# airl-iisc/MRFP

Measured on AMD Instinct MI355X. Metric: train images/sec, higher is better.
Workload: dtype bf16; 1 GPU; resnet-101 DeepLabV3+ + MRFP+ (HRFP+NP+ on, HRFP re-drawn every step), 768x768, 16 images/GPU, fwd+bwd+SGD, synthetic 19-class, random-init weights; global_batch=16, parallelism=dp1

## Files before the change

### include/mrfp_hip.h

```cpp
#ifndef MRFP_HIP_H
#define MRFP_HIP_H

#include <stdint.h>

#ifdef __cplusplus
extern "C" {
#endif

typedef enum { MRFP_F32 = 0, MRFP_BF16 = 1, MRFP_F16 = 2 } mrfp_dtype;

int mrfp_version(void);
const char* mrfp_last_error(void);

int64_t mrfp_stats_nslab(int64_t B, int64_t Ho);

int mrfp_stats_fwd(const void* x, int dtype, int64_t B, int64_t Ho, int64_t Wo, int64_t C,
                   int64_t Hs, int64_t Ws, const int32_t* tabH, const int32_t* tabW,
                   float* ws, void* stream);

int mrfp_stats_bwd(const void* dy, const void* x, const void* y, const float* mean,
                   const float* fA, const float* fS, int per_image, int dtype, int64_t B, int64_t Ho, int64_t Wo, int64_t C,
                   int64_t Hs, int64_t Ws, const int32_t* tabH, const int32_t* tabW,
                   float* ws, void* stream);
int mrfp_stats_bwd_mask(const void* dy, const void* x, const void* mask, const float* mean, int per_image, int dtype, int64_t B,
// ... 117 lines not shown
                  int64_t sstride, const void* addend, float* colstats, void* stream);
int mrfp_conv_fwd_act(const void* x, const void* wpack, const float* bias, void* y, int dtype,
                      int64_t B, int64_t H, int64_t W, int64_t C, int64_t N, int64_t ldy, int64_t R, int64_t S,
                      int64_t Ho, int64_t Wo, int64_t stride, int64_t pad_h, int64_t pad_w, int64_t dil,
                      int64_t sstride, const void* addend, int act, void* stream);
int mrfp_pack_weight_folded(const float* w, void* wf, const float* conv_bias, const float* bn_weight, const float* bn_bias,
                            const float* running_mean, const float* running_var, float eps, float* bias_out, int dtype,
                            int64_t N, int64_t C, int64_t R, int64_t S, int64_t Npad, int64_t Cpad, void* stream);
int mrfp_pack_weights_folded_batched(const void* jobs, const int64_t* prefix, int64_t njobs, int64_t total, int dtype, void* stream);
int mrfp_conv_stats_layout(int dtype, int64_t B, int64_t H, int64_t W, int64_t C, int64_t N, int64_t ldy, int64_t R, int64_t S,
                           int64_t Ho, int64_t Wo, int64_t stride, int64_t pad_h, int64_t pad_w, int64_t dil, int64_t sstride, int wstats,
                           int64_t* out);
int64_t mrfp_conv_stats_block_rows(int dtype, int64_t B, int64_t H, int64_t W, int64_t C, int64_t N, int64_t R, int64_t S, int64_t Ho,
                                   int64_t Wo, int64_t stride, int64_t pad_h, int64_t pad_w, int64_t dil, int64_t sstride);
int mrfp_conv_single_launch(int64_t B, int64_t image_bytes);
int mrfp_conv_fwd_wstats(const void* x, const void* wpack, const float* bias, void* y, int dtype,
                         int64_t B, int64_t H, int64_t W, int64_t C, int64_t N, int64_t ldy, int64_t R, int64_t S,
                         int64_t Ho, int64_t Wo, int64_t stride, int64_t pad_h, int64_t pad_w, int64_t dil,
                         const uint8_t* rowweight, float* colstats, void* stream);
int mrfp_conv_fwd_gated(const void* x, const void* wpack, const float* bias, void* y, int dtype,
                        int64_t B, int64_t H, int64_t W, int64_t C, int64_t N, int64_t ldy, int64_t R, int64_t S,
                        int64_t Ho, int64_t Wo, int64_t stride, int64_t pad_h, int64_t pad_w, int64_t dil,
                        int64_t sstride, const void* addend, const void* addend_mask, void* stream);
int mrfp_debug_clock_stamps(int family, uint64_t* out, int64_t n);
int64_t mrfp_conv_wgrad_ws_bytes(int64_t M, int64_t N, int64_t Q);
int mrfp_conv_wgrad(const void* x, const void* dy, float* dw, void* ws, int dtype,
                    int64_t B, int64_t H, int64_t W, int64_t C, int64_t Ctrue, int64_t N, int64_t ldn,
                    int64_t R, int64_t S, int64_t Ho, int64_t Wo, int64_t stride, int64_t pad_h, int64_t pad_w,
                    int64_t dil, void* stream);
int64_t mrfp_conv_wgrad_group_max(void);
int64_t mrfp_conv_wgrad_grouped_ws_bytes(int64_t M, int64_t N, int64_t Q, int64_t count);
int mrfp_conv_wgrad_plan(int dtype, int64_t B, int64_t H, int64_t W, int64_t C, int64_t N, int64_t ldn, int64_t R, int64_t S, int64_t Ho,
                         int64_t Wo, int64_t stride, int64_t pad_h, int64_t pad_w, int64_t dil, int64_t count, int64_t* out);
int mrfp_conv_wgrad_grouped(const void* const* xs, const void* const* dys, float* const* dws, int64_t count, void* ws, int dtype,
                            int64_t B, int64_t H, int64_t W, int64_t C, int64_t Ctrue, int64_t N, int64_t ldn,
                            int64_t R, int64_t S, int64_t Ho, int64_t Wo, int64_t stride, int64_t pad_h, int64_t pad_w,
                            int64_t dil, void* stream);
int mrfp_nchw_to_nhwc_pad(const float* x, void* y, int dtype, int64_t B, int64_t C, int64_t H, int64_t W,
                          int64_t Cpad, void* stream);

int mrfp_sgd_step(float* p, const float* g, float* m, int64_t n, float lr, float momentum,
                  float weight_decay, float gscale, int first, void* stream);

int64_t mrfp_grad_check_nblocks(int64_t n);
int mrfp_grad_check(const float* g, int64_t n, float gscale, void* ws, void* state, int dynamic, float growth,
                    float backoff, int growth_interval, float max_norm, void* stream);
// ... 70 lines not shown
```

### mrfp_amd/conv.py

```python
from __future__ import annotations

import collections
import ctypes
import os as _os
import warnings
import weakref
from typing import Any, NamedTuple, Optional

import torch

from . import _lib
from ._lib import call, dt, ptr, stream
from .ops import CL, GRAD_DEFERRED, _chk, channel_sums, empty_cl, grad_sink, notify_grad, wgrad_workspace, zeros_cl
from .ops import _inside_autograd_engine as _in_backward

_PACKS = {}
FUSE_STATS = [_os.environ.get("MRFP_FUSE_STATS", "1") != "0"]


class ConvStats(NamedTuple):
    final: torch.Tensor
    final_count: int
    elements: int
    rows: torch.Tensor
    row_blocks: int
    block_rows: int
    resize_plan: Any
    version: int


WSTATS = [_os.environ.get("MRFP_WSTATS", "1") != "0"]
WSTATS_HITS = [0]
_EPOCH = [0]


def invalidate_packs():
    _EPOCH[0] += 1
# ... 546 lines not shown
        else:
            call("mrfp_conv_fwd", ptr(x), ptr(pk.wf), ptr(pk.bias), ptr(y), dt(x), B, H, W, Cphys, Nphys, Nphys, R, S,
                 Ho, Wo, stride, pad_h, pad_w, dil, 1, None, ptr(stats), stream())
        ctx.save_for_backward(x, weight, bias)
        ctx.cfg = (stride, pad_h, pad_w, dil, Nphys, Ho, Wo)
        ctx.set_materialize_grads(False)
        if want_skip:
            return y, x.view_as(x)
        return y

    @staticmethod
    def backward(ctx, dy, dskip=None):
        x, weight, bias = ctx.saved_tensors
        cell = getattr(ctx, "_mrfp_cell", None)
        if cell is not None and cell[1]:
            g = getattr(dskip, "_mrfp_gate", None) if dskip is not None else None
            if g is None or g[1] != dskip._version:
                raise _lib.MrfpHipError("a gated skip gradient reached its convolution without its gate: the skip alias was "
                                        "also consumed by an operator outside mrfp_amd.ops (set MRFP_GATED_SKIP=0)")
            cell[1] = False
        if dy is None:
            return (ungate(dskip),) + (None,) * 10
        stride, pad_h, pad_w, dil, Nphys, Ho, Wo = ctx.cfg
        dy = _chk(dy, "dy")
        B, Cphys, H, W = x.shape
        N, C, R, S = weight.shape
        dx = dw = db = None
        if ctx.needs_input_grad[0]:
            pk = get_pack(weight, bias, x.dtype, Cphys, Nphys)
            dx = empty_cl(B, Cphys, H, W, x.dtype, x.device)
            gate = None
            if dskip is not None:
                g = getattr(dskip, "_mrfp_gate", None)
                if g is not None:
                    if (g[1] == dskip._version and dskip.dtype == x.dtype and x.element_size() == 2
                            and Cphys % 8 == 0 and dskip.shape == dx.shape and dskip.is_contiguous(memory_format=CL)):
                        gate = g[0]
                    else:
                        dskip = ungate(dskip)
                dskip = _chk(dskip, "dskip")
                if dskip.dtype != x.dtype:
                    dskip = dskip.to(x.dtype)
            _lib.NOTE[0] = (N, C)
            if gate is not None:
                call("mrfp_conv_fwd_gated", ptr(dy), ptr(pk.wd), None, ptr(dx), dt(dy), B, Ho, Wo, Nphys, Cphys, Cphys, R, S, H, W,
                     1, dil * (R - 1) - pad_h, dil * (S - 1) - pad_w, dil, stride, ptr(dskip), ptr(gate), stream())
                GATED_SKIP_HITS[0] += 1
            else:
                call("mrfp_conv_fwd", ptr(dy), ptr(pk.wd), None, ptr(dx), dt(dy), B, Ho, Wo, Nphys, Cphys, Cphys, R, S, H, W,
                     1, dil * (R - 1) - pad_h, dil * (S - 1) - pad_w, dil, stride, ptr(dskip), None, stream())
        if ctx.needs_input_grad[1]:
            sig = (x.dtype, B, H, W, Cphys, C, N, Nphys, R, S, Ho, Wo, stride, pad_h, pad_w, dil)
            sink = grad_sink(weight)
            side = _WGRADS.stream(x.device) if sink is not None else None
            if sink is not None and GROUP_WGRAD[0] and L_single(B, H, W, Cphys, Ho, Wo, Nphys, x.element_size()):
                _WGRADS.submit(sig, x, dy, sink, weight)
            elif side is not None:
                _WGRADS.ensure_callback()
                _launch_wgrads(sig, [(x, dy, sink)], side)
                notify_grad(weight)
            else:
                dw = sink if sink is not None else torch.empty((N, C, R, S), dtype=torch.float32, device=x.device)
                _launch_wgrads(sig, [(x, dy, dw)], None)
                if sink is not None:
                    notify_grad(weight)
                    dw = None
                elif dw.dtype != weight.dtype:
# ... 99 lines not shown
    R, S = weight.shape[2], weight.shape[3]
    Ho, Wo = _out_size(H, R, st, ph, dl), _out_size(W, S, st, pw, dl)
    L = _lib.lib()
    single = bool(L.mrfp_conv_single_launch(B, H * W * Cphys * x.element_size()))
    plan, wtab, stats = stat_resize, None, None
    if plan is not None and WSTATS[0] and FUSE_STATS[0] and single and (plan.Hs, plan.Ws) == (Ho, Wo) and R * S > 1:
        wtab = plan.multiplicity(B)
    if wtab is not None or (bias is None and FUSE_STATS[0] and single):
        lay = (ctypes.c_int64 * 5)()
        rc = L.mrfp_conv_stats_layout(dt(x), B, H, W, Cphys, Nphys, Nphys, R, S, Ho, Wo, st, ph, pw, dl, 1, int(wtab is not None), lay)
        if rc != 0:
            raise _lib.MrfpHipError("mrfp_conv_stats_layout failed (%d): %s" % (rc, L.mrfp_last_error().decode()))
        nblk, rb, rows, first, cnt = lay
        stats = torch.empty(rows * 2 * Nphys, dtype=torch.float32, device=x.device)
    if _WGRADS.callback_queued and not _in_backward():
        _WGRADS.drop_stale()
    out = _Conv2d.apply(x, weight, bias, st, ph, pw, dl, Nphys, want_skip, stats, wtab)
    y, skip = out if want_skip else (out, None)
    if skip is not None:
        skip._mrfp_skip_alias = True
        skip._mrfp_uses = [0, False]
        if y.grad_fn is not None:
            y.grad_fn._mrfp_cell = skip._mrfp_uses
    if stats is not None and (phys_out is not None or Nphys == N):
        final = stats[first * 2 * Nphys:(first + cnt) * 2 * Nphys]
        if wtab is not None:
            y._mrfp_colstats = ConvStats(final, cnt, B * plan.Ho * plan.Wo, stats, nblk, 0, plan, y._version)
        else:
            y._mrfp_colstats = ConvStats(final, cnt, B * Ho * Wo, stats, nblk, rb, None, y._version)
    if phys_out is None and Nphys != N:
        y = y[:, :N].contiguous(memory_format=CL)
    return (y, skip) if want_skip else y
```

### mrfp_amd/csrc/conv_pwk.hip

```cpp
#include "conv_common.hpp"

namespace mrfp {

#if MRFP_CLOCK_STAMP
__device__ unsigned long long g_phase_pwk[kStampSlots][2];
int stamps_pwk(unsigned long long* out, int n) { return hipMemcpyFromSymbol(out, HIP_SYMBOL(g_phase_pwk), (size_t)n * 16) == hipSuccess ? 0 : -1; }
struct PhaseClock {
    unsigned long long acc[8];
    unsigned long long cnt[8];
    unsigned long long last, t0, r0;
    static __device__ __forceinline__ unsigned long long now() {
        const unsigned long long t = __builtin_amdgcn_s_memtime();
        __builtin_amdgcn_s_waitcnt(0xC07F);
        return t;
    }
    __device__ __forceinline__ void start() {
#pragma unroll
        for (int k = 0; k < 8; ++k) { acc[k] = 0; cnt[k] = 0; }
        r0 = __builtin_amdgcn_s_memrealtime();
        last = t0 = now();
    }
    template <int K> __device__ __forceinline__ void lap() {
        const unsigned long long t = now();
        acc[K] += t - last;
// ... 18 lines not shown
#else
int stamps_pwk(unsigned long long*, int) { return -1; }
#define PH_START()
#define PH_LAP(k)
#define PH_FLUSH(w)
#endif


struct PkP {
    const char* x;
    const char* w;
    char* y;
    const char* addend;
    const unsigned char* addend_mask;
    float* colstats;
    int M, N, ldy;
    int tiles;
    int panels;
    int chunks;
    unsigned xbytes, wbytes, ybytes;
};

constexpr int kPkRows = 48;

template <typename T, int KQ, int NST, bool STATS, bool ADD, int ACT = 0>
__global__ __launch_bounds__(256, (KQ <= 2 ? 2 : 1)) void conv1x1_longk_kernel(PkP p) {
    constexpr int ROWB = KQ * 512;
    constexpr int STAGE = 4 * kPkRows * 128;
    constexpr int NP = 6;
    extern __shared__ __attribute__((aligned(16))) char smem[];
    const int t = threadIdx.x, lane = t & 63;
    const int wave = __builtin_amdgcn_readfirstlane(t >> 6);
    const int l15 = lane & 15, lq = lane >> 4;
    const unsigned lds0 = (unsigned)(size_t)(__attribute__((address_space(3))) char*)smem;
    const i32x4 xw = rsrc_words(p.x, p.xbytes);
    const __amdgpu_buffer_rsrc_t wr = __builtin_amdgcn_make_buffer_rsrc((void*)p.w, 0, (int)p.wbytes, 0x00020000);
    const __amdgpu_buffer_rsrc_t yr = __builtin_amdgcn_make_buffer_rsrc((void*)p.y, 0, (int)p.ybytes, 0x00020000);
    const __amdgpu_buffer_rsrc_t ar = __builtin_amdgcn_make_buffer_rsrc((void*)(p.addend ? p.addend : p.y), 0, (int)p.ybytes, 0x00020000);

    const int b = blockIdx.x, xcd = b & 7, rest = b >> 3;
    const int panel = rest % p.panels, chunk = xcd + 8 * (rest / p.panels);
    if (chunk >= p.chunks) return;
    const int per = (p.tiles + p.chunks - 1) / p.chunks;
    const int t0 = chunk * per, t1 = min(p.tiles, t0 + per);
    if (t0 >= t1) return;
    const int n0 = panel * 128 + wave * 32, nl = n0 + 8 * lq;
// ... 120 lines not shown
            u32x4 dv;
            dv.x = v.x; dv.y = v.y; dv.z = v.z; dv.w = v.w;
            __builtin_amdgcn_raw_buffer_store_b128(dv, yr, (int)(ok ? ((unsigned)m * (unsigned)p.ldy + (unsigned)nl) * 2u : kOOB), 0, 0);
        }
    }
    if constexpr (STATS) {
        float* out = p.colstats + (size_t)chunk * 2 * p.ldy;
#pragma unroll
        for (int u = 0; u < 8; ++u) {
            cs[u] = row16_sum(cs[u]);
            cq[u] = row16_sum(cq[u]);
        }
        if (l15 == 0 && nl < p.N) {
#pragma unroll
            for (int u = 0; u < 8; ++u) {
                out[nl + u] = cs[u];
                out[p.ldy + nl + u] = cq[u];
            }
        }
    }
}

constexpr int kPk2Rows = 32;

template <typename T, bool STATS, bool ADD, int ACT = 0>
__global__ __launch_bounds__(512, 2) void conv1x1_longk2_kernel(PkP p) {
    constexpr int ROWB = 2048;
    constexpr int QTR = 4 * kPk2Rows * 128;
    constexpr int PAIR = 2 * QTR;
    constexpr int NST = 4;
    constexpr int NP = 4;
    extern __shared__ __attribute__((aligned(16))) char smem[];
    char* const exch = smem + NST * PAIR;
    const int t = threadIdx.x, lane = t & 63;
    const int wave = __builtin_amdgcn_readfirstlane(t >> 6);
    const int grp = wave >> 2, wq = wave & 3;
    const int l15 = lane & 15, lq = lane >> 4;
    const unsigned lds0 = (unsigned)(size_t)(__attribute__((address_space(3))) char*)smem;
    const i32x4 xw = rsrc_words(p.x, p.xbytes);
    const __amdgpu_buffer_rsrc_t wr = __builtin_amdgcn_make_buffer_rsrc((void*)p.w, 0, (int)p.wbytes, 0x00020000);
    const __amdgpu_buffer_rsrc_t yr = __builtin_amdgcn_make_buffer_rsrc((void*)p.y, 0, (int)p.ybytes, 0x00020000);
    const __amdgpu_buffer_rsrc_t ar = __builtin_amdgcn_make_buffer_rsrc((void*)(p.addend ? p.addend : p.y), 0, (int)p.ybytes, 0x00020000);

    const int b = blockIdx.x, xcd = b & 7, rest = b >> 3;
    const int panel = rest % p.panels, chunk = xcd + 8 * (rest / p.panels);
    if (chunk >= p.chunks) return;
    const int per = (p.tiles + p.chunks - 1) / p.chunks;
    const int t0 = chunk * per, t1 = min(p.tiles, t0 + per);
    if (t0 >= t1) return;
    const int n0 = panel * 128 + wq * 32, nl = n0 + 8 * lq;
    const int total = (t1 - t0) * 2;
    PH_START();

    unsigned src[NP];
#pragma unroll
    for (int j = 0; j < NP; ++j) {
        const int pi = j * 8 + wave, qs = pi >> 4, wi = pi & 15, kb = wi >> 2, r8 = wi & 3;
        const int row = r8 * 8 + (lane >> 3);
        const int ch = (lane & 7) ^ ((row >> 1) & 7);
        src[j] = (unsigned)row * (unsigned)ROWB + (unsigned)(qs * 1024 + kb * 128 + ch * 16);
    }
    auto issue = [&](int h) {
        const int tile = t0 + (h >> 1), sst = h & 1;
        const unsigned base = (unsigned)tile * (unsigned)(kPk2Rows * ROWB) + (unsigned)(sst * 512);
        const unsigned sbase = lds0 + (unsigned)((h % NST) * PAIR);
#pragma unroll
        for (int j = 0; j < NP; ++j) {
            const int pi = j * 8 + wave, qs = pi >> 4, wi = pi & 15, kb = wi >> 2, r8 = wi & 3;
            dma16_async(xw, sbase + (unsigned)(qs * QTR + kb * (kPk2Rows * 128) + r8 * 1024), base + src[j]);
        }
    };
#pragma unroll
    for (int h = 0; h < NST - 1; ++h)
        if (h < total) issue(h);

    uint4 fw[16][2];
#pragma unroll
    for (int ks = 0; ks < 16; ++ks)
#pragma unroll
        for (int j = 0; j < 2; ++j) {
            const int n = n0 + 8 * (l15 >> 2) + 4 * j + (l15 & 3);
            fw[ks][j] = bload(wr, n < p.N ? (unsigned)n * (unsigned)ROWB + (unsigned)(grp * 1024 + ks * 64 + lq * 16) : kOOB);
        }
#pragma unroll
    for (int ks = 0; ks < 16; ++ks)
#pragma unroll
        for (int j = 0; j < 2; ++j) settle(fw[ks][j]);
    PH_LAP(0);

    float cs[8], cq[8];
#pragma unroll
    for (int u = 0; u < 8; ++u) { cs[u] = 0.f; cq[u] = 0.f; }

    int h = 0;
    for (int tile = t0; tile < t1; ++tile) {
        f32x4 acc[2][2];
        uint4 av[2];
        unsigned am[2] = {0xffu, 0xffu};
#pragma unroll
        for (int sst = 0; sst < 2; ++sst, ++h) {
            if (h + NST - 1 <= total) dma_wait<(NST - 2) * NP>();
            else dma_wait<0>();
            __builtin_amdgcn_s_barrier();
            PH_LAP(1);
            if (h + NST - 1 < total) issue(h + NST - 1);
            PH_LAP(2);
            if constexpr (ADD) {
                if (sst == 0 && grp == 0) {
#pragma unroll
                    for (int rb = 0; rb < 2; ++rb) {
                        const int m = tile * kPk2Rows + rb * 16 + l15;
                        const bool ok = m < p.M && nl < p.N;
                        av[rb] = bload(ar, ok ? ((unsigned)m * (unsigned)p.ldy + (unsigned)nl) * 2u : kOOB);
                        am[rb] = (p.addend_mask && ok) ? p.addend_mask[((size_t)m * p.ldy + nl) >> 3] : 0xffu;
                    }
                }
            }
            const char* st = smem + (h % NST) * PAIR + grp * QTR;
            uint4 fx[2][2];
            auto read_x = [&](int ks, uint4 (&f)[2]) {
                const char* ab = st + (ks >> 1) * (kPk2Rows * 128);
                const int ch = (ks & 1) * 4 + lq;
#pragma unroll
                for (int rb = 0; rb < 2; ++rb) f[rb] = *reinterpret_cast<const uint4*>(ab + lds_off(rb * 16 + l15, ch));
            };
            read_x(0, fx[0]);
#pragma unroll
            for (int ks = 0; ks < 8; ++ks) {
                if (ks + 1 < 8) read_x(ks + 1, fx[(ks + 1) & 1]);
                __builtin_amdgcn_sched_barrier(0);
#pragma unroll
                for (int rb = 0; rb < 2; ++rb)
#pragma unroll
                    for (int j = 0; j < 2; ++j) {
                        if (sst == 0 && ks == 0) {
                            const f32x4 z = {0.f, 0.f, 0.f, 0.f};
                            acc[rb][j] = z;
                        }
                        Mma16<T>::run(acc[rb][j], fw[sst * 8 + ks][j], fx[ks & 1][rb]);
                    }
                __builtin_amdgcn_sched_barrier(0);
            }
            PH_LAP(3);
        }
        f32x4* ex = reinterpret_cast<f32x4*>(exch) + (wq * 4) * 64 + lane;
        if (grp == 1) {
#pragma unroll
            for (int rb = 0; rb < 2; ++rb)
#pragma unroll
                for (int j = 0; j < 2; ++j) ex[(rb * 2 + j) * 64] = acc[rb][j];
        }
        asm volatile("s_waitcnt lgkmcnt(0)" ::: "memory");
        __builtin_amdgcn_s_barrier();
        if (grp == 0) {
#pragma unroll
            for (int rb = 0; rb < 2; ++rb) {
#pragma unroll
                for (int j = 0; j < 2; ++j) {
                    const f32x4 o = ex[(rb * 2 + j) * 64];
#pragma unroll
                    for (int e = 0; e < 4; ++e) acc[rb][j][e] += o[e];
                }
                const int m = tile * kPk2Rows + rb * 16 + l15;
                const bool ok = m < p.M && nl < p.N;
// ... 87 lines not shown

template <typename T, bool STATS, bool ADD, int ACT = 0>
static int pwk2_launch(const ConvP& c, hipStream_t st) {
    constexpr int lds = 4 * 2 * 4 * kPk2Rows * 128 + kPk2Rows * 128 * 4;
    static bool attr_set = false;
    if (!attr_set) {
        (void)hipFuncSetAttribute(reinterpret_cast<const void*>(&conv1x1_longk2_kernel<T, STATS, ADD, ACT>),
                                  hipFuncAttributeMaxDynamicSharedMemorySize, lds);
        attr_set = true;
    }
    PkP p;
    p.x = c.x; p.w = c.w; p.y = c.y; p.addend = c.addend; p.addend_mask = c.addend_mask; p.colstats = c.colstats;
    p.M = c.M; p.N = c.N; p.ldy = c.ldy;
    p.tiles = (c.M + kPk2Rows - 1) / kPk2Rows;
    p.panels = (c.N + 127) / 128;
    p.chunks = pwk_chunks(c.M, c.N, 2048);
    const int chunks = (p.chunks + 7) / 8 * 8;
    p.xbytes = c.xbytes; p.wbytes = c.wbytes; p.ybytes = (unsigned)((int64_t)c.M * c.ldy * 2);
    hipLaunchKernelGGL((conv1x1_longk2_kernel<T, STATS, ADD, ACT>), dim3((unsigned)(p.panels * chunks)), dim3(512), lds, st, p);
    MRFP_LAUNCH_CHECK();
    return 0;
}

template <typename T, int KQ, bool STATS, bool ADD, int ACT = 0>
static int pwk_launch(const ConvP& c, hipStream_t st) {
    constexpr int NST = KQ <= 2 ? 3 : 6;
    constexpr int lds = NST * 4 * kPkRows * 128;
    static bool attr_set = false;
    if (!attr_set) {
        (void)hipFuncSetAttribute(reinterpret_cast<const void*>(&conv1x1_longk_kernel<T, KQ, NST, STATS, ADD, ACT>),
                                  hipFuncAttributeMaxDynamicSharedMemorySize, lds);
        attr_set = true;
    }
    PkP p;
    p.x = c.x; p.w = c.w; p.y = c.y; p.addend = c.addend; p.addend_mask = c.addend_mask; p.colstats = c.colstats;
    p.M = c.M; p.N = c.N; p.ldy = c.ldy;
    p.tiles = (c.M + kPkRows - 1) / kPkRows;
    p.panels = (c.N + 127) / 128;
    p.chunks = pwk_chunks(c.M, c.N, c.C * 2);
    const int chunks = (p.chunks + 7) / 8 * 8;
    p.xbytes = c.xbytes; p.wbytes = c.wbytes; p.ybytes = (unsigned)((int64_t)c.M * c.ldy * 2);
    hipLaunchKernelGGL((conv1x1_longk_kernel<T, KQ, NST, STATS, ADD, ACT>), dim3((unsigned)(p.panels * chunks)), dim3(256), lds, st, p);
    MRFP_LAUNCH_CHECK();
    return 0;
}
template <typename T, int KQ>
// ... 6 lines not shown
    if (p.colstats) return pwk_launch<T, KQ, true, false>(p, st);
    if (p.addend) return pwk_launch<T, KQ, false, true>(p, st);
    return pwk_launch<T, KQ, false, false>(p, st);
}
template <typename T>
static int pwk_run_t(const ConvP& p, hipStream_t st, int act) {
    const int kq = p.C * 2 / 512;
    static const int two = env_switch("MRFP_CONV_PWK2", 1);
    if (kq == 4 && two) {
        if (act != 0) {
            if (p.colstats || p.addend_mask) return -1;
            if (act == 1) return p.addend ? pwk2_launch<T, false, true, 1>(p, st) : pwk2_launch<T, false, false, 1>(p, st);
            return p.addend ? pwk2_launch<T, false, true, 2>(p, st) : pwk2_launch<T, false, false, 2>(p, st);
        }
        if (p.colstats) return pwk2_launch<T, true, false>(p, st);
        if (p.addend) return pwk2_launch<T, false, true>(p, st);
        return pwk2_launch<T, false, false>(p, st);
    }
    return kq == 2 ? pwk_pick<T, 2>(p, st, act) : kq == 4 ? pwk_pick<T, 4>(p, st, act) : pwk_pick<T, 5>(p, st, act);
}
int pwk_run(const ConvP& p, bool is_f16, hipStream_t st, int act) { return is_f16 ? pwk_run_t<f16>(p, st, act) : pwk_run_t<bf16>(p, st, act); }

}
```

### mrfp_amd/ops.py

```python
from __future__ import annotations

import math
import os
import weakref
from functools import lru_cache
from typing import Optional, Tuple

import numpy as np
import torch

from . import _lib
from ._lib import call, dt, ptr, stream

CL = torch.channels_last

GRAD_NOTIFY = [None]
GRAD_DEFERRED = set()


def wgrad_workspace(M, N, Q, device, n=1):
    return torch.empty(int(_lib.lib().mrfp_conv_wgrad_grouped_ws_bytes(M, N, Q, n)), dtype=torch.uint8, device=device)


def grad_sink(param):
    if param is not None and getattr(param, "_mrfp_direct", False) and param.grad is not None \
            and param.grad.dtype == torch.float32 and param.grad.is_contiguous():
        return param.grad
    return None


def notify_grad(param):
    if GRAD_NOTIFY[0] is not None:
        GRAD_NOTIFY[0](param)


def to_cl(x: torch.Tensor) -> torch.Tensor:
    if x.dim() != 4:
        raise ValueError("expected a 4-D activation, got %s" % (tuple(x.shape),))
    return x.contiguous(memory_format=CL)


def empty_cl(B, C, H, W, dtype, device) -> torch.Tensor:
    return torch.empty((B, C, H, W), dtype=dtype, device=device, memory_format=CL)


def zeros_cl(B, C, H, W, dtype, device) -> torch.Tensor:
    return torch.zeros((B, H, W, C), dtype=dtype, device=device).permute(0, 3, 1, 2)


def _chk(x: torch.Tensor, name="x") -> torch.Tensor:
    if not x.is_cuda:
        raise _lib.MrfpHipError("%s must live on the GPU (got %s): the HIP path has no CPU fallback" % (name, x.device))
    uses = getattr(x, "_mrfp_uses", None)
    if uses is not None:
        uses[0] += 1
    if x.dim() != 4 or not x.is_contiguous(memory_format=CL):
        x = to_cl(x)
    return x


def _f32(t: Optional[torch.Tensor]) -> Optional[torch.Tensor]:
    if t is None:
        return None
    return t.detach().float().contiguous()


def nearest_out_size(in_size: int, scale: float) -> int:
    return int(math.floor(float(in_size) * scale))


def _nearest_table(in_size: int, out_size: int, scale: Optional[float]) -> np.ndarray:
    s = np.float32(1.0 / scale) if scale is not None else np.float32(in_size) / np.float32(out_size)
    src = np.floor(np.arange(out_size, dtype=np.float32) * s).astype(np.int64)
    return np.minimum(src, in_size - 1).astype(np.int32)


def _inverse_table(tab: np.ndarray, in_size: int) -> np.ndarray:
    lo = np.searchsorted(tab, np.arange(in_size), side="left")
# ... 206 lines not shown
    SYNC_BN_CALLS[0] += 1
    total = 0
    if count:
        key = (int(count), dist.get_world_size(group))
        total = _SYNC_BN_COUNTS.get(key)
        if total is None:
            total = _SYNC_BN_COUNTS[key] = int(round(tot[2 * C].item()))
        else:
            flag = _SYNC_BN_FLAG.get(ws.device)
            if flag is None:
                flag = _SYNC_BN_FLAG[ws.device] = torch.zeros(1, dtype=torch.int32, device=ws.device)
            flag.add_((tot[2 * C:2 * C + 1] != float(total)).to(torch.int32))
    return torch.stack([hi, lo]).contiguous(), total


ACT_NONE, ACT_RELU, ACT_RELU6 = 0, 1, 2
GATED_BN_HITS = [0]
GATED_BN = [os.environ.get("MRFP_GATED_BN", "1") != "0"]
RELU6_GATE_HITS = [0]


def _keeps_sign_mask(x, relu, res, plan):
    return bool(relu and res is not None and plan is None and SIGN_MASK[0] and x.element_size() == 2 and x.shape[1] % 8 == 0)


class _BatchNormAct(torch.autograd.Function):

    @staticmethod
    def forward(ctx, x, weight, bias, running_mean, running_var, res, training, momentum, eps, act, plan, may_sync, stats):
        relu, relu6 = act == ACT_RELU, act == ACT_RELU6
        if relu6 and (res is not None or plan is not None):
            raise _lib.MrfpHipError("BatchNorm + ReLU6 takes no residual and no resize plan")
        x = _chk(x)
        res = _chk(res, "res") if res is not None else None
        B, Ho, Wo, C, Hs, Ws, *_ = _geom(x, plan)
        dev = x.device
        w32, b32 = _f32(weight), _f32(bias)
        coef = torch.empty(4 * C, dtype=torch.float32, device=dev)
        mean, invstd, A, S = coef[0:C], coef[C:2 * C], coef[2 * C:3 * C], coef[3 * C:4 * C]
        if training:
            fused = _serving_colstats(x, C, B * Ho * Wo, plan, False)
            if fused is not None:
                ws, nb_, nslab = fused.final, 1, fused.final_count
            else:
                nslab, ws = _stats_fwd(x, plan)
                nb_ = B
            count = B * Ho * Wo
            ctx.sync = _sync_bn_group() if may_sync else None
            if ctx.sync is not None:
                ws, count = _allreduce_stats(ws, nb_ * nslab, C, count, ctx.sync)
                nb_, nslab = 1, 2
            ctx.count = count
            call("mrfp_bn_finalize", ptr(ws), nb_, nslab, count, C, ptr(w32), ptr(b32), float(eps),
                 float(momentum), ptr(running_mean), ptr(running_var), ptr(mean), ptr(invstd), ptr(A), ptr(S), stream())
        else:
            ctx.sync, ctx.count = None, B * Ho * Wo
            call("mrfp_bn_eval_coef", C, ptr(w32), ptr(b32), ptr(running_mean), ptr(running_var), float(eps),
                 ptr(A), ptr(S), stream())
            if x.requires_grad or (weight is not None and weight.requires_grad):
                mean.copy_(running_mean)
                torch.rsqrt(running_var.float() + eps, out=invstd)
        ctx.plan, ctx.act, ctx.training, ctx.has_res = plan, act, training, res is not None
        ctx.keep_y = relu and res is not None
        ctx.remask = relu and res is None
        ctx.ymask = _keeps_sign_mask(x, relu, res, plan)
        ctx.gate_skip = bool(ctx.ymask and GATED_SKIP[0] and getattr(res, "_mrfp_skip_alias", False))
        ctx.gate_ok = bool(act == ACT_NONE and res is None and plan is None and training and x.element_size() == 2 and C % 8 == 0)
        ctx.alias_uses = getattr(res, "_mrfp_uses", None)
        keep = None
        if relu6:
            y = empty_cl(B, C, Ho, Wo, x.dtype, dev)
            keep = torch.empty((B * Ho * Wo * C + 7) // 8, dtype=torch.uint8, device=dev)
            call("mrfp_affine_fwd_relu6_mask", ptr(x), ptr(y), ptr(keep), dt(x), B * Ho * Wo, C, ptr(A), ptr(S), stream())
        elif ctx.ymask:
            y = empty_cl(B, C, Ho, Wo, x.dtype, dev)
            keep = torch.empty(B * Ho * Wo * C // 8, dtype=torch.uint8, device=dev)
            call("mrfp_affine_fwd_relu_mask", ptr(x), ptr(res), ptr(y), ptr(keep), dt(x), B, Ho, Wo, C, ptr(A), ptr(S), 0, stream())
        else:
            y = _affine_fwd(x, res, A, S, False, relu, plan, stats=stats)
            if ctx.keep_y:
                keep = y
        ctx.wparam, ctx.bparam = weight, bias
        ctx.save_for_backward(x, keep, w32, mean, invstd, A, S)
        return y

    @staticmethod
    def backward(ctx, dy):
        x, keep, w32, mean, invstd, A, S = ctx.saved_tensors
        gate = None
        cell = getattr(ctx, "_mrfp_cell", None)
        g = getattr(dy, "_mrfp_gate", None)
# ... 37 lines not shown
        out = torch.empty(5 * C, dtype=torch.float32, device=dy.device)
        dw, db, P, Q, R = (out[i * C:(i + 1) * C] for i in range(5))
        dw = _grad_dest(ctx.wparam, ctx.needs_input_grad[1], dw)
        db = _grad_dest(ctx.bparam, ctx.needs_input_grad[2], db)
        call("mrfp_bn_bwd_finalize", ptr(ws), B, nslab, B * Ho * Wo, C, ptr(w32), ptr(mean), ptr(invstd),
             ptr(dw), ptr(db), ptr(P), ptr(Q), ptr(R), stream())
        if ctx.sync is not None:
            gws, _ = _allreduce_stats(ws, B * nslab, C, 0, ctx.sync)
            call("mrfp_bn_bwd_finalize", ptr(gws), 1, 2, ctx.count, C, ptr(w32), ptr(mean), ptr(invstd), None, None,
                 ptr(P), ptr(Q), ptr(R), stream())
        if not ctx.training:
            Q.zero_()
            R.zero_()
        if mask is not None:
            dx = empty_cl(B, C, Ho, Wo, dy.dtype, dy.device)
            dres = dres_out = None
            if ctx.ymask:
                if ctx.gate_skip and ctx.needs_input_grad[5] and ctx.alias_uses is not None and ctx.alias_uses[0] == 1:
                    dres = dy.view_as(dy)
                    dres._mrfp_gate = (mask, dres._version)
                    ctx.alias_uses[1] = True
                else:
                    dres = dres_out = empty_cl(B, C, Ho, Wo, dy.dtype, dy.device)
            call("mrfp_affine_bwd_mask", ptr(dy), ptr(x), ptr(mask), ptr(dx), ptr(dres_out), dt(dy), B, Ho, Wo, C, ptr(P), ptr(Q),
                 ptr(R), 0, stream())
        else:
            dx, dres = _affine_bwd(dy, x, y, P, Q, R, False, plan, ctx.has_res, x, fA, fS)
        return (dx, _grad_result(ctx.wparam, dw), _grad_result(ctx.bparam, db), None, None, dres) + (None,) * 7


RUNNING_STATS_EPOCH = [0]


def batch_norm_act(x, weight, bias, running_mean, running_var, *, training, momentum=0.1, eps=1e-5,
                   relu=False, res=None, plan=None, emit_stats=False):
    if training and running_mean is not None:
        RUNNING_STATS_EPOCH[0] += 1
    ps = _planestats_rows(x, emit_stats and plan is None and not _keeps_sign_mask(x, relu, res, plan))
    y = _BatchNormAct.apply(x, weight, bias, running_mean, running_var, res, training, momentum, eps,
                            ACT_RELU if relu else ACT_NONE, plan, True, ps[1] if ps is not None else None)
    _tag_planestats(y, ps)
    if (GATED_BN[0] and GATED_SKIP[0] and SIGN_MASK[0] and not relu and res is None and plan is None and training and y.grad_fn is not None
            and y.element_size() == 2 and y.shape[1] % 8 == 0):
        y._mrfp_skip_alias = True
        y._mrfp_uses = [0, False]
        y.grad_fn._mrfp_cell = y._mrfp_uses
    return y

# ... 1142 lines not shown
```

Measured before the change: 310.0 images/sec.

## Fuse BN-ReLU-mask backward into the following 1x1 conv's dgrad prologue

Defers the masked BN+ReLU backward elementwise pass by attaching a pending descriptor to its dx tensor. When that tensor reaches the backward of a 1x1 stride-1 K=1024 convolution, a new variant of the long-K pointwise kernel computes the BN backward on the fly while loading dy. It writes the materialized gradient once and feeds it straight into LDS for the dgrad GEMM. This removes a separate full read and write pass of the activation gradient. In exchange it adds a register-staged prologue with fewer LDS stages, use-counting and tracking machinery, and a fallback path that materializes the gradient when another op consumes it.

Result: no change. 309.9 images/sec (-0.0%).

```diff
diff --git a/include/mrfp_hip.h b/include/mrfp_hip.h
--- a/include/mrfp_hip.h
+++ b/include/mrfp_hip.h
@@ -163,6 +163,9 @@
                         int64_t B, int64_t H, int64_t W, int64_t C, int64_t N, int64_t ldy, int64_t R, int64_t S,
                         int64_t Ho, int64_t Wo, int64_t stride, int64_t pad_h, int64_t pad_w, int64_t dil,
                         int64_t sstride, const void* addend, const void* addend_mask, void* stream);
+int mrfp_conv_pw_tail_served(int dtype, int64_t B, int64_t H, int64_t W, int64_t C, int64_t N);
+int mrfp_conv_pw_tail_bwd(const void* dy, const void* x3, const void* mask, const float* P, const float* Q, const float* R, void* dx3,
+                          const void* wpack, void* y, int dtype, int64_t B, int64_t H, int64_t W, int64_t C, int64_t N, void* stream);
 int mrfp_debug_clock_stamps(int family, uint64_t* out, int64_t n);
 int64_t mrfp_conv_wgrad_ws_bytes(int64_t M, int64_t N, int64_t Q);
 int mrfp_conv_wgrad(const void* x, const void* dy, float* dw, void* ws, int dtype,
diff --git a/mrfp_amd/conv.py b/mrfp_amd/conv.py
--- a/mrfp_amd/conv.py
+++ b/mrfp_amd/conv.py
@@ -13,6 +13,7 @@
 from ._lib import call, dt, ptr, stream
 from .ops import CL, GRAD_DEFERRED, _chk, channel_sums, empty_cl, grad_sink, notify_grad, wgrad_workspace, zeros_cl
 from .ops import _inside_autograd_engine as _in_backward
+from . import ops
 
 _PACKS = {}
 FUSE_STATS = [_os.environ.get("MRFP_FUSE_STATS", "1") != "0"]
@@ -605,9 +606,18 @@
         if dy is None:
             return (ungate(dskip),) + (None,) * 10
         stride, pad_h, pad_w, dil, Nphys, Ho, Wo = ctx.cfg
-        dy = _chk(dy, "dy")
         B, Cphys, H, W = x.shape
         N, C, R, S = weight.shape
+        pend = None
+        tail = getattr(ctx, "_mrfp_tail_cell", None)
+        if tail is not None and tail[1]:
+            tail[1] = False
+            if getattr(dy, "_mrfp_pending", None) is None:
+                raise _lib.MrfpHipError("a pending tail gradient reached its convolution without its operands: the convolution's output "
+                                        "was also consumed by an operator outside mrfp_amd.ops (set MRFP_FUSE_TAIL_PW=0)")
+            if ctx.needs_input_grad[0] and dskip is None and dy.dtype == x.dtype and dy.is_contiguous(memory_format=CL):
+                pend = ops.take_pending(dy)
+        dy = _chk(dy, "dy")
         dx = dw = db = None
         if ctx.needs_input_grad[0]:
             pk = get_pack(weight, bias, x.dtype, Cphys, Nphys)
@@ -625,7 +635,11 @@
                 if dskip.dtype != x.dtype:
                     dskip = dskip.to(x.dtype)
             _lib.NOTE[0] = (N, C)
-            if gate is not None:
+            if pend is not None:
+                call("mrfp_conv_pw_tail_bwd", ptr(pend.dy), ptr(pend.x), ptr(pend.mask), ptr(pend.P), ptr(pend.Q), ptr(pend.R), ptr(dy),
+                     ptr(pk.wd), ptr(dx), dt(dy), B, Ho, Wo, Nphys, Cphys, stream())
+                ops.TAIL_PW_HITS[0] += 1
+            elif gate is not None:
                 call("mrfp_conv_fwd_gated", ptr(dy), ptr(pk.wd), None, ptr(dx), dt(dy), B, Ho, Wo, Nphys, Cphys, Cphys, R, S, H, W,
                      1, dil * (R - 1) - pad_h, dil * (S - 1) - pad_w, dil, stride, ptr(dskip), ptr(gate), stream())
                 GATED_SKIP_HITS[0] += 1
@@ -771,6 +785,10 @@
         skip._mrfp_uses = [0, False]
         if y.grad_fn is not None:
             y.grad_fn._mrfp_cell = skip._mrfp_uses
+    if (ops.FUSE_TAIL_PW[0] and not want_skip and bias is None and R == 1 and S == 1 and st == 1 and ph == 0 and pw == 0
+            and y.grad_fn is not None and x.requires_grad and L.mrfp_conv_pw_tail_served(dt(x), B, Ho, Wo, Nphys, Cphys) == 1):
+        y._mrfp_tail_cell = [0, False, weakref.ref(y)]
+        y.grad_fn._mrfp_tail_cell = y._mrfp_tail_cell
     if stats is not None and (phys_out is not None or Nphys == N):
         final = stats[first * 2 * Nphys:(first + cnt) * 2 * Nphys]
         if wtab is not None:
diff --git a/mrfp_amd/csrc/conv_pwk.hip b/mrfp_amd/csrc/conv_pwk.hip
--- a/mrfp_amd/csrc/conv_pwk.hip
+++ b/mrfp_amd/csrc/conv_pwk.hip
@@ -64,6 +64,17 @@
 };
 
 constexpr int kPkRows = 48;
+
+struct PkPre : PkP {
+    const char* a;
+    const unsigned char* mask_in;
+    char* out;
+    unsigned char* mask_out;
+    const float* c0;
+    const float* c1;
+    const float* c2;
+    unsigned mbytes;
+};
 
 template <typename T, int KQ, int NST, bool STATS, bool ADD, int ACT = 0>
 __global__ __launch_bounds__(256, (KQ <= 2 ? 2 : 1)) void conv1x1_longk_kernel(PkP p) {
@@ -230,13 +241,29 @@
 }
 
 constexpr int kPk2Rows = 32;
-
-template <typename T, bool STATS, bool ADD, int ACT = 0>
-__global__ __launch_bounds__(512, 2) void conv1x1_longk2_kernel(PkP p) {
+#ifndef MRFP_PWK_PRE_DEPTH
+#define MRFP_PWK_PRE_DEPTH 1
+#endif
+
+template <typename T> __device__ __forceinline__ unsigned pack_rt(float a, float b) {
+    const T x = from_f<T>(a), y = from_f<T>(b);
+    unsigned short xs, ys;
+    __builtin_memcpy(&xs, &x, 2);
+    __builtin_memcpy(&ys, &y, 2);
+    return (unsigned)xs | ((unsigned)ys << 16);
+}
+__device__ __forceinline__ void lds_publish() {
+    asm volatile("s_waitcnt lgkmcnt(0)" ::: "memory");
+    __builtin_amdgcn_s_barrier();
+    asm volatile("" ::: "memory");
+}
+
+template <typename T, bool STATS, bool ADD, int ACT = 0, int PRE = 0>
+__global__ __launch_bounds__(512, 2) void conv1x1_longk2_kernel(typename std::conditional<PRE != 0, PkPre, PkP>::type p) {
     constexpr int ROWB = 2048;
     constexpr int QTR = 4 * kPk2Rows * 128;
     constexpr int PAIR = 2 * QTR;
-    constexpr int NST = 4;
+    constexpr int NST = PRE ? 2 : 4;
     constexpr int NP = 4;
     extern __shared__ __attribute__((aligned(16))) char smem[];
     char* const exch = smem + NST * PAIR;
@@ -261,12 +288,14 @@
     PH_START();
 
     unsigned src[NP];
-#pragma unroll
-    for (int j = 0; j < NP; ++j) {
-        const int pi = j * 8 + wave, qs = pi >> 4, wi = pi & 15, kb = wi >> 2, r8 = wi & 3;
-        const int row = r8 * 8 + (lane >> 3);
-        const int ch = (lane & 7) ^ ((row >> 1) & 7);
-        src[j] = (unsigned)row * (unsigned)ROWB + (unsigned)(qs * 1024 + kb * 128 + ch * 16);
+    if constexpr (PRE == 0) {
+#pragma unroll
+        for (int j = 0; j < NP; ++j) {
+            const int pi = j * 8 + wave, qs = pi >> 4, wi = pi & 15, kb = wi >> 2, r8 = wi & 3;
+            const int row = r8 * 8 + (lane >> 3);
+            const int ch = (lane & 7) ^ ((row >> 1) & 7);
+            src[j] = (unsigned)row * (unsigned)ROWB + (unsigned)(qs * 1024 + kb * 128 + ch * 16);
+        }
     }
     auto issue = [&](int h) {
         const int tile = t0 + (h >> 1), sst = h & 1;
@@ -278,9 +307,104 @@
             dma16_async(xw, sbase + (unsigned)(qs * QTR + kb * (kPk2Rows * 128) + r8 * 1024), base + src[j]);
         }
     };
-#pragma unroll
-    for (int h = 0; h < NST - 1; ++h)
-        if (h < total) issue(h);
+    if constexpr (PRE == 0) {
+#pragma unroll
+        for (int h = 0; h < NST - 1; ++h)
+            if (h < total) issue(h);
+    }
+
+    const int pqs = wave & 1, pkb = lane >> 4, pch = lane & 7, prow = (wave >> 1) * 8 + ((lane >> 3) & 1);
+    const unsigned poff = (unsigned)prow * (unsigned)ROWB + (unsigned)(pqs * 1024 + pkb * 128 + pch * 16);
+    float* const coef = reinterpret_cast<float*>(exch + kPk2Rows * 128 * 4);
+    constexpr int DEPTH = MRFP_PWK_PRE_DEPTH;
+    uint4 ra[DEPTH][4], rb[DEPTH][4];
+    unsigned rm[DEPTH][4];
+    auto pre_load = [&](int h, uint4 (&A)[4], uint4 (&B)[4], unsigned (&Mk)[4]) {
+        if constexpr (PRE != 0) {
+            const __amdgpu_buffer_rsrc_t x0 = __builtin_amdgcn_make_buffer_rsrc((void*)p.x, 0, (int)p.xbytes, 0x00020000);
+            const __amdgpu_buffer_rsrc_t x1 = __builtin_amdgcn_make_buffer_rsrc((void*)p.a, 0, (int)p.xbytes, 0x00020000);
+            const unsigned base = (unsigned)(t0 + (h >> 1)) * (unsigned)(kPk2Rows * ROWB) + (unsigned)((h & 1) * 512) + poff;
+#pragma unroll
+            for (int j = 0; j < 4; ++j) {
+                const unsigned o = h < total ? base + (unsigned)(j * 2 * ROWB) : kOOB;
+                A[j] = bload(x0, o);
+                B[j] = bload(x1, o);
+                if constexpr (PRE == 2) {
+                    const __amdgpu_buffer_rsrc_t mr = __builtin_amdgcn_make_buffer_rsrc((void*)p.mask_in, 0, (int)p.mbytes, 0x00020000);
+                    Mk[j] = __builtin_amdgcn_raw_buffer_load_b8(mr, (int)(o >> 4), 0, 0);
+                }
+            }
+        }
+    };
+    auto pre_stage = [&](int h, const uint4 (&A)[4], const uint4 (&B)[4], const unsigned (&Mk)[4]) {
+        if constexpr (PRE != 0) {
+            const __amdgpu_buffer_rsrc_t orr = __builtin_amdgcn_make_buffer_rsrc((void*)p.out, 0, (int)p.xbytes, 0x00020000);
+            const int tile = t0 + (h >> 1);
+            const int c = (h & 1) * 256 + pqs * 512 + pkb * 64 + pch * 8;
+            const unsigned base = (unsigned)tile * (unsigned)(kPk2Rows * ROWB) + (unsigned)((h & 1) * 512) + poff;
+            const bool store = panel == 0 && h < total;
+            char* const slot = smem + (h % NST) * PAIR + pqs * QTR + pkb * (kPk2Rows * 128);
+            float k0[8], k1[8], k2[8];
+#pragma unroll
+            for (int i = 0; i < 8; ++i) {
+                k0[i] = coef[c + i];
+                k1[i] = coef[1024 + c + i];
+                k2[i] = PRE == 2 ? coef[2048 + c + i] : 0.f;
+            }
+#pragma unroll
+            for (int j = 0; j < 4; ++j) {
+                const int row = prow + 2 * j;
+                float a[8], b[8], v[8];
+                unpack2<T>(A[j].x, a[0], a[1]);
+                unpack2<T>(A[j].y, a[2], a[3]);
+                unpack2<T>(A[j].z, a[4], a[5]);
+                unpack2<T>(A[j].w, a[6], a[7]);
+                unpack2<T>(B[j].x, b[0], b[1]);
+                unpack2<T>(B[j].y, b[2], b[3]);
+                unpack2<T>(B[j].z, b[4], b[5]);
+                unpack2<T>(B[j].w, b[6], b[7]);
+                unsigned bits = 0;
+#pragma unroll
+                for (int i = 0; i < 8; ++i) {
+                    if constexpr (PRE == 1) {
+                        float y = a[i] * k0[i] + k1[i];
+                        y += b[i];
+                        y = y > 0.f ? y : 0.f;
+                        v[i] = y;
+                        bits |= (to_f(from_f<T>(y)) > 0.f ? 1u : 0u) << i;
+                    } else {
+                        const float d = ((Mk[j] >> i) & 1u) ? a[i] : 0.f;
+                        v[i] = k0[i] * d + (k1[i] * b[i] + k2[i]);
+                    }
+                }
+                uint4 o;
+                o.x = pack_rt<T>(v[0], v[1]);
+                o.y = pack_rt<T>(v[2], v[3]);
+                o.z = pack_rt<T>(v[4], v[5]);
+                o.w = pack_rt<T>(v[6], v[7]);
+                const unsigned go = store ? base + (unsigned)(j * 2 * ROWB) : kOOB;
+                u32x4 dv;
+                dv.x = o.x; dv.y = o.y; dv.z = o.z; dv.w = o.w;
+                __builtin_amdgcn_raw_buffer_store_b128(dv, orr, (int)go, 0, 0);
+                if constexpr (PRE == 1) {
+                    const __amdgpu_buffer_rsrc_t mr = __builtin_amdgcn_make_buffer_rsrc((void*)p.mask_out, 0, (int)p.mbytes, 0x00020000);
+                    __builtin_amdgcn_raw_buffer_store_b8((unsigned char)bits, mr, (int)(go >> 4), 0, 0);
+                }
+                if (tile * kPk2Rows + row >= p.M) o = make_uint4(0u, 0u, 0u, 0u);
+                *reinterpret_cast<uint4*>(slot + lds_off(row, pch)) = o;
+            }
+        }
+    };
+    if constexpr (PRE != 0) {
+        for (int i = t; i < 768; i += 512) {
+            const float* s = i < 256 ? p.c0 : i < 512 ? p.c1 : p.c2;
+            float4 v = make_float4(0.f, 0.f, 0.f, 0.f);
+            if (s) v = *reinterpret_cast<const float4*>(s + (i & 255) * 4);
+            *reinterpret_cast<float4*>(coef + i * 4) = v;
+        }
+#pragma unroll
+        for (int d = 0; d < DEPTH; ++d) pre_load(d, ra[d], rb[d], rm[d]);
+    }
 
     uint4 fw[16][2];
 #pragma unroll
@@ -294,6 +418,11 @@
     for (int ks = 0; ks < 16; ++ks)
 #pragma unroll
         for (int j = 0; j < 2; ++j) settle(fw[ks][j]);
+    if constexpr (PRE != 0) {
+        lds_publish();
+        pre_stage(0, ra[0], rb[0], rm[0]);
+        pre_load(DEPTH, ra[0], rb[0], rm[0]);
+    }
     PH_LAP(0);
 
     float cs[8], cq[8];
@@ -307,12 +436,23 @@
         unsigned am[2] = {0xffu, 0xffu};
 #pragma unroll
         for (int sst = 0; sst < 2; ++sst, ++h) {
-            if (h + NST - 1 <= total) dma_wait<(NST - 2) * NP>();
-            else dma_wait<0>();
-            __builtin_amdgcn_s_barrier();
-            PH_LAP(1);
-            if (h + NST - 1 < total) issue(h + NST - 1);
-            PH_LAP(2);
+            if constexpr (PRE == 0) {
+                if (h + NST - 1 <= total) dma_wait<(NST - 2) * NP>();
+                else dma_wait<0>();
+                __builtin_amdgcn_s_barrier();
+                PH_LAP(1);
+                if (h + NST - 1 < total) issue(h + NST - 1);
+                PH_LAP(2);
+            } else {
+                lds_publish();
+                PH_LAP(1);
+                if (grp == 0) {
+                    const int d = (sst + 1) % DEPTH;
+                    pre_stage(h + 1, ra[d], rb[d], rm[d]);
+                    pre_load(h + 1 + DEPTH, ra[d], rb[d], rm[d]);
+                }
+                PH_LAP(2);
+            }
             if constexpr (ADD) {
                 if (sst == 0 && grp == 0) {
 #pragma unroll
@@ -348,6 +488,13 @@
                         Mma16<T>::run(acc[rb][j], fw[sst * 8 + ks][j], fx[ks & 1][rb]);
                     }
                 __builtin_amdgcn_sched_barrier(0);
+            }
+            if constexpr (PRE != 0) {
+                if (grp == 1) {
+                    const int d = (sst + 1) % DEPTH;
+                    pre_stage(h + 1, ra[d], rb[d], rm[d]);
+                    pre_load(h + 1 + DEPTH, ra[d], rb[d], rm[d]);
+                }
             }
             PH_LAP(3);
         }
@@ -481,6 +628,33 @@
     return 0;
 }
 
+static bool pwk_tail_served(int dtype, int64_t B, int64_t H, int64_t W, int64_t C, int64_t N) {
+    static const int two = env_switch("MRFP_CONV_PWK2", 1);
+    if (!two || (dtype != MRFP_BF16 && dtype != MRFP_F16) || B <= 0 || H <= 0 || W <= 0 || C != 1024 || N < 128 || (N & 127) != 0) return false;
+    const int64_t M = B * H * W;
+    if (M * 2048 >= (int64_t)kOOB) return false;
+    ConvP c{};
+    c.B = (int)B; c.H = c.Ho = (int)H; c.W = c.Wo = (int)W; c.C = (int)C; c.N = c.ldy = (int)N;
+    c.R = c.S = c.stride = c.sstride = c.dil = 1;
+    c.M = (int)M;
+    return pwk_applicable(c, 2);
+}
+
+template <typename T, int PRE>
+static int pwk2_pre_launch(const PkPre& q, hipStream_t st) {
+    constexpr int lds = 2 * 2 * 4 * kPk2Rows * 128 + kPk2Rows * 128 * 4 + 3 * 1024 * 4;
+    static bool attr_set = false;
+    if (!attr_set) {
+        (void)hipFuncSetAttribute(reinterpret_cast<const void*>(&conv1x1_longk2_kernel<T, PRE == 1, false, 0, PRE>),
+                                  hipFuncAttributeMaxDynamicSharedMemorySize, lds);
+        attr_set = true;
+    }
+    const int chunks = (q.chunks + 7) / 8 * 8;
+    hipLaunchKernelGGL((conv1x1_longk2_kernel<T, PRE == 1, false, 0, PRE>), dim3((unsigned)(q.panels * chunks)), dim3(512), lds, st, q);
+    MRFP_LAUNCH_CHECK();
+    return 0;
+}
+
 template <typename T, int KQ, bool STATS, bool ADD, int ACT = 0>
 static int pwk_launch(const ConvP& c, hipStream_t st) {
     constexpr int NST = KQ <= 2 ? 3 : 6;
@@ -533,3 +707,34 @@
 int pwk_run(const ConvP& p, bool is_f16, hipStream_t st, int act) { return is_f16 ? pwk_run_t<f16>(p, st, act) : pwk_run_t<bf16>(p, st, act); }
 
 }
+
+using namespace mrfp;
+
+extern "C" {
+
+int mrfp_conv_pw_tail_served(int dtype, int64_t B, int64_t H, int64_t W, int64_t C, int64_t N) {
+    return pwk_tail_served(dtype, B, H, W, C, N) ? 1 : 0;
+}
+
+int mrfp_conv_pw_tail_bwd(const void* dy, const void* x3, const void* mask, const float* P, const float* Q, const float* R, void* dx3,
+                          const void* wpack, void* y, int dtype, int64_t B, int64_t H, int64_t W, int64_t C, int64_t N, void* stream) {
+    MRFP_CHECK(dy && x3 && mask && P && Q && R && dx3 && wpack && y, "conv_pw_tail_bwd: bad arguments");
+    MRFP_CHECK(dtype == MRFP_BF16 || dtype == MRFP_F16, "conv_pw_tail_bwd: 16-bit activations only (dtype %d)", dtype);
+    MRFP_CHECK(pwk_tail_served(dtype, B, H, W, C, N),
+               "conv_pw_tail_bwd: not served (1x1, stride 1, K = 1024, N %% 128 == 0, a launch of the long-K pointwise kernel): see mrfp_conv_pw_tail_served");
+    MRFP_CHECK(aligned16(dy) && aligned16(x3) && aligned16(dx3) && aligned16(wpack) && aligned16(y) && aligned16(P) && aligned16(Q) && aligned16(R),
+               "conv_pw_tail_bwd: operands must be 16-byte aligned");
+    PkPre q{};
+    q.x = (const char*)dy; q.w = (const char*)wpack; q.y = (char*)y;
+    q.M = (int)(B * H * W); q.N = (int)N; q.ldy = (int)N;
+    q.tiles = (q.M + kPk2Rows - 1) / kPk2Rows;
+    q.panels = (int)(N / 128);
+    q.chunks = pwk_chunks(q.M, q.N, 2048);
+    q.xbytes = (unsigned)((int64_t)q.M * 2048); q.wbytes = (unsigned)(N * 2048); q.ybytes = (unsigned)((int64_t)q.M * N * 2);
+    q.a = (const char*)x3; q.mask_in = (const unsigned char*)mask; q.out = (char*)dx3;
+    q.c0 = P; q.c1 = Q; q.c2 = R;
+    q.mbytes = (unsigned)((int64_t)q.M * 128);
+    return dtype == MRFP_F16 ? pwk2_pre_launch<f16, 2>(q, (hipStream_t)stream) : pwk2_pre_launch<bf16, 2>(q, (hipStream_t)stream);
+}
+
+}
diff --git a/mrfp_amd/ops.py b/mrfp_amd/ops.py
--- a/mrfp_amd/ops.py
+++ b/mrfp_amd/ops.py
@@ -46,6 +46,48 @@
 
 def zeros_cl(B, C, H, W, dtype, device) -> torch.Tensor:
     return torch.zeros((B, H, W, C), dtype=dtype, device=device).permute(0, 3, 1, 2)
+
+
+FUSE_TAIL_PW = [os.environ.get("MRFP_FUSE_TAIL_PW", "1") != "0"]
+TAIL_PW_HITS = [0]
+_TAKEN = object()
+
+
+class PendingTail:
+    __slots__ = ("dy", "x", "mask", "P", "Q", "R", "version")
+
+    def __init__(self, dy, x, mask, P, Q, R, version):
+        self.dy, self.x, self.mask, self.P, self.Q, self.R, self.version = dy, x, mask, P, Q, R, version
+
+
+def _pending(t):
+    pend = getattr(t, "_mrfp_pending", None) if t is not None else None
+    if pend is None or pend is _TAKEN:
+        return pend
+    if pend.version != t._version:
+        raise _lib.MrfpHipError("a pending tail gradient was modified in place before it was applied")
+    return pend
+
+
+def take_pending(t):
+    pend = _pending(t)
+    if pend is _TAKEN:
+        raise _lib.MrfpHipError("a pending tail gradient was consumed twice")
+    if pend is None:
+        raise _lib.MrfpHipError("not a pending tail gradient")
+    t._mrfp_pending = _TAKEN
+    return pend
+
+
+def materialize(t):
+    pend = _pending(t)
+    if pend is None or pend is _TAKEN:
+        return t
+    del t._mrfp_pending
+    B, C, H, W = t.shape
+    call("mrfp_affine_bwd_mask", ptr(pend.dy), ptr(pend.x), ptr(pend.mask), ptr(t), None, dt(t), B, H, W, C, ptr(pend.P), ptr(pend.Q),
+         ptr(pend.R), 0, stream())
+    return t
 
 
 def _chk(x: torch.Tensor, name="x") -> torch.Tensor:
@@ -54,6 +96,11 @@
     uses = getattr(x, "_mrfp_uses", None)
     if uses is not None:
         uses[0] += 1
+    tail = getattr(x, "_mrfp_tail_cell", None)
+    if tail is not None:
+        tail[0] += 1
+    if getattr(x, "_mrfp_pending", None) is not None:
+        materialize(x)
     if x.dim() != 4 or not x.is_contiguous(memory_format=CL):
         x = to_cl(x)
     return x
@@ -306,6 +353,11 @@
 
 def _keeps_sign_mask(x, relu, res, plan):
     return bool(relu and res is not None and plan is None and SIGN_MASK[0] and x.element_size() == 2 and x.shape[1] % 8 == 0)
+
+
+def _unobserved(ref):
+    t = ref() if ref is not None else None
+    return t is None or not (t._backward_hooks or t.retains_grad)
 
 
 class _BatchNormAct(torch.autograd.Function):
@@ -351,6 +403,7 @@
         ctx.gate_skip = bool(ctx.ymask and GATED_SKIP[0] and getattr(res, "_mrfp_skip_alias", False))
         ctx.gate_ok = bool(act == ACT_NONE and res is None and plan is None and training and x.element_size() == 2 and C % 8 == 0)
         ctx.alias_uses = getattr(res, "_mrfp_uses", None)
+        ctx.tail_cell = getattr(x, "_mrfp_tail_cell", None) if (ctx.ymask and FUSE_TAIL_PW[0]) else None
         keep = None
         if relu6:
             y = empty_cl(B, C, Ho, Wo, x.dtype, dev)
@@ -434,8 +487,14 @@
                     ctx.alias_uses[1] = True
                 else:
                     dres = dres_out = empty_cl(B, C, Ho, Wo, dy.dtype, dy.device)
-            call("mrfp_affine_bwd_mask", ptr(dy), ptr(x), ptr(mask), ptr(dx), ptr(dres_out), dt(dy), B, Ho, Wo, C, ptr(P), ptr(Q),
-                 ptr(R), 0, stream())
+            cell = ctx.tail_cell
+            if (cell is not None and FUSE_TAIL_PW[0] and cell[0] == 1 and not cell[1] and dres_out is None and mask is keep
+                    and dy.dtype == x.dtype and ctx.needs_input_grad[0] and _unobserved(cell[2])):
+                dx._mrfp_pending = PendingTail(dy, x, mask, P, Q, R, dx._version)
+                cell[1] = True
+            else:
+                call("mrfp_affine_bwd_mask", ptr(dy), ptr(x), ptr(mask), ptr(dx), ptr(dres_out), dt(dy), B, Ho, Wo, C, ptr(P), ptr(Q),
+                     ptr(R), 0, stream())
         else:
             dx, dres = _affine_bwd(dy, x, y, P, Q, R, False, plan, ctx.has_res, x, fA, fS)
         return (dx, _grad_result(ctx.wparam, dw), _grad_result(ctx.bparam, db), None, None, dres) + (None,) * 7
```
